# MG-RAST/Shock

Measured on AMD Instinct MI355X. Metric: device-resident index-build GiB/s + Mrecords/s, 10 GiB FASTQ, 1/2/4/8 GPU, higher is better.
Workload: dtype u8; 1 GPU; fastq record index, 10 GiB synthetic node file in HBM (BASELINE configs[1]); records=30969274, bytes=10737418240, tile=16384, parallelism=single slab, exchange=none (one slab: no collective)

## Files before the change

shock_amd/core.py:

```python
from __future__ import annotations

import ctypes
import os
import weakref
from dataclasses import dataclass, field

import numpy as np

from . import _lib as L


@dataclass
class IndexResult:
    count: int
    fmt: str | None
    status: int
    err: bytes | None
    rows: np.ndarray | None = None
    timings: dict = field(default_factory=dict)
    path: int = 0
    reruns: int = 0
    state_out: int = 0
    term_code: int = 0
    flags: int = 0
# ... 157 lines not shown
    def chunkrecord_buffer(self, data: "DeviceBuffer", n: int, rows: "DeviceBuffer", fmt=None,
                           chunk: int = 0) -> IndexResult:
        return self.chunkrecord_device(data.ptr, n, rows.ptr, rows.nbytes // 16, fmt, chunk)

    @staticmethod
    def chunkrecord_capacity(n: int, chunk: int = 0) -> int:
        return n // ((chunk or 1048576) - 32767) + 2

    def column_device(self, d_data: int, n: int, column: int, d_rows: int, row_cap: int) -> IndexResult:
        res = L.Result()
        rc = self._lib.shockidx_column_device(self._h, d_data, n, column, d_rows, row_cap, ctypes.byref(res))
        return _result(res, rc)

    def column_buffer(self, data: "DeviceBuffer", n: int, column: int, rows: "DeviceBuffer") -> IndexResult:
        return self.column_device(data.ptr, n, column, rows.ptr, rows.nbytes // 16)

    def column_fd(self, fd: int, size: int, column: int) -> IndexResult:
        res = L.Result()
        rows_p = ctypes.POINTER(ctypes.c_uint64)()
        rc = self._lib.shockidx_column_fd(self._h, fd, size, column, ctypes.byref(rows_p), ctypes.byref(res))
        rows = _take_rows(rows_p, int(res.count)) if rows_p else None
        return _result(res, rc, rows)

    def column_host(self, data, column: int) -> IndexResult:
        data = bytes(data)
        n = len(data)
        d_in = self.alloc(n + 64)
        d_in.upload(data)
        cap = 1024
        d_rows = self.alloc(16 * cap)
        try:
            r = self.column_buffer(d_in, n, column, d_rows)
            if r.status == L.ESPACE:
                d_rows.free()
                cap = r.count
                d_rows = self.alloc(16 * cap)
                r = self.column_buffer(d_in, n, column, d_rows)
            if r.status == L.OK:
                r.rows = d_rows.rows(r.count) if r.count else np.zeros((0, 2), np.uint64)
            return r
        finally:
            d_in.free()
            d_rows.free()

    def set_dev_cap(self, nbytes: int) -> None:
        rc = self._lib.shockidx_ctx_set_dev_cap(self._h, int(nbytes))
        if rc != 0:
            raise L.ShockIdxError(rc, "shockidx_ctx_set_dev_cap failed")

    def trim(self, keep_bytes: int = 0) -> None:
        rc = self._lib.shockidx_ctx_trim(self._h, int(keep_bytes))
        if rc != L.OK:
            raise L.ShockIdxError(rc, "shockidx_ctx_trim failed")

    def workspace_bytes(self) -> int:
        return int(self._lib.shockidx_ctx_workspace_bytes(self._h))

    def alloc(self, nbytes: int, node: bool = False) -> "DeviceBuffer":
        return DeviceBuffer(self, nbytes, node)

    def sync(self):
        rc = self._lib.shockidx_sync(self._h)
        if rc != L.OK:
            raise L.ShockIdxError(rc, "shockidx_sync failed")

    @property
    def stream(self) -> int:
        return self._lib.shockidx_stream(self._h)

    def subset_index(self, d_ids: int, ids_len: int, d_parent: int, parent_count: int, ilength: int, d_rows: int,
                     rows_cap: int, d_runs: int, runs_cap: int) -> SubsetResult:
        r = L.SubsetResult()
        rc = self._lib.shockidx_subset_index(self._h, d_ids, ids_len, d_parent, parent_count, ilength, d_rows, rows_cap,
                                             d_runs, runs_cap, ctypes.byref(r))
        return _sub_result(r, rc)

    def subset_gather(self, d_data: int, data_len: int, d_runs: int, nruns: int, d_out: int,
                      out_cap: int) -> SubsetResult:
        r = L.SubsetResult()
        rc = self._lib.shockidx_subset_gather(self._h, d_data, data_len, d_runs, nruns, d_out, out_cap,
                                              ctypes.byref(r))
        return _sub_result(r, rc)

    def subset_node(self, d_ids: int, ids_len: int, d_parent: int, parent_count: int, ilength: int, d_rows: int,
                    rows_cap: int, d_runs: int, runs_cap: int, d_data: int, data_len: int, d_out: int,
                    out_cap: int) -> SubsetResult:
        r = L.SubsetResult()
        rc = self._lib.shockidx_subset_node(self._h, d_ids, ids_len, d_parent, parent_count, ilength, d_rows, rows_cap,
                                            d_runs, runs_cap, d_data, data_len, d_out, out_cap, ctypes.byref(r))
        return _sub_result(r, rc)

    def subset_host(self, ids, parent_rows, ilength=None, data=None) -> SubsetResult:
        ids = bytes(ids)
        par = np.ascontiguousarray(parent_rows, dtype=np.uint64).reshape(-1, 2)
        n = par.shape[0]
        il = n if ilength is None else int(ilength)
        d_ids = self.alloc(len(ids) + 64)
        d_ids.upload(ids)
        d_par = self.alloc(16 * n + 64)
        if n:
            d_par.upload(par.tobytes())
        cap = max(1, len(ids) // 2 + 2)
        d_rows = self.alloc(16 * cap)
        d_runs = self.alloc(16 * cap)
        r = self.subset_index(d_ids.ptr, len(ids), d_par.ptr, n, il, d_rows.ptr, cap, d_runs.ptr, cap)
        if r.status in (L.OK, L.EFORMAT):
# ... 338 lines not shown
```

shock_amd/csrc/sidx_build.cpp:

```cpp
#include <errno.h>
#include <hip/hip_runtime.h>
#include <stdio.h>
#include <stdlib.h>
#include <string.h>
#include <sys/mman.h>
#include <unistd.h>

#include <atomic>
#include <mutex>
#include <vector>

#include "../../include/shockidx.h"
#include "sidx_common.hpp"
#include "sidx_subset.hpp"
#include "sidx_launch.hpp"
#include "sidx_host.hpp"

using namespace sidx;

namespace sidx_host {

CopyPool::CopyPool(int n) : nt_(n) {
  for (int i = 0; i < n; ++i) th_.emplace_back([this, i] { run(i); });
}
// ... 167 lines not shown
}

int run_index(shockidx_ctx *c, const uint8_t *d_data, u64 n, int kfmt, u64 *d_rows, u64 row_cap,
              hipStream_t s, DevResult *dr, shockidx_result *res, const SlabGeom *geom, bool general,
              const int *gate) {
  const u64 ntiles = n ? (n + TILE - 1) / TILE : 1;
  if (ntiles >= (1ull << KEY_TILE_BITS)) return set_msg(res, SHOCKIDX_EINVAL, "input too large for one slab");
  if (int rc = ensure_tiles(c, ntiles, res)) return rc;
  const TilePass pass = choose_pass(c, kfmt, n, geom, general);
  if (pass != TP_TWO_PASS) {
    const u64 words = sidx_tile_stage_words(pass, ntiles, c->tiles_grid);
    c->d_tile_stage.node = ws_contig(2);
    if (int rc = c->d_tile_stage.ensure(words, res)) return rc;
    if (int rc = c->d_tile_words.ensure(ntiles * FQ_TILE_WORDS, res)) return rc;
    if (pass == TP_FQ && c->want_spans)
      if (int rc = c->d_fqlines.ensure(ntiles * 3 * (TILE / 64), res)) return rc;
  }
  if (getenv("SHOCKIDX_TIMING") && !c->d_timing) {
    HIPCHK(hipMalloc(&c->d_timing, 9 * 8 * 65536), "hipMalloc(timing)");
  }
  if (c->slots_dirty) {
    HIPCHK(hipMemsetAsync(c->d_small + SMALL_BADKEY, 0xFF, 16, s), "slot reset");
    HIPCHK(hipMemsetAsync(c->d_small + SMALL_COUNTERS, 0, 2 * 4 * NCOUNTERS, s), "slot reset");
    c->slots_dirty = false;
  }
  if (++c->epoch > EPOCH_MASK) {
    HIPCHK(hipMemsetAsync(c->d_status, 0, c->d_status.bytes(), s), "status clear");
    c->epoch = 2;
  }
  c->slots_dirty = true;
  const u32 slot = c->epoch & 1;
  SlabParams p;
  memset(&p, 0, sizeof p);
  p.data = d_data;
  p.n = n;
  p.end = geom ? geom->end : n;
  p.front = geom ? geom->front : 0;
  p.base = geom ? geom->base : 0;
  p.state_in = geom ? geom->state_in : 0;
  p.row_base = geom ? geom->row_base : 0;
  p.summary = geom ? (u64 *)geom->d_summary : nullptr;
  p.row_cap = row_cap;
  p.rows = d_rows;
  auto status_array = [c](StatusArray a) { return c->d_status + (u64)a * c->tiles_cap(); };
  p.status = status_array(SA_STATUS);
  p.pcnt = status_array(SA_PCNT);
  p.ppre = status_array(SA_PPRE);
  for (int i = 0; i < 2; ++i) p.scan_look[i] = status_array((StatusArray)(SA_LOOK0 + i));
  p.tile_agg = status_array(SA_TILE_AGG);
  p.tile_excl = status_array(SA_TILE_EXCL);
  p.pgrid = c->tiles_grid < ntiles ? c->tiles_grid : (u32)ntiles;
  p.fix = general ? nullptr : c->d_fix.get();
  p.fixcap = (u32)c->tiles_cap();
  p.badkey = (u64 *)(c->d_small + SMALL_BADKEY + 8 * slot);
  p.badkey_next = (u64 *)(c->d_small + SMALL_BADKEY + 8 * (slot ^ 1));
  p.detail = c->d_detail;
  p.counters = (u32 *)(c->d_small + SMALL_COUNTERS + 4 * NCOUNTERS * slot);
  p.counters_next = (u32 *)(c->d_small + SMALL_COUNTERS + 4 * NCOUNTERS * (slot ^ 1));
  p.ntiles = (u32)ntiles;
  p.epoch = c->epoch;
  p.seq = geom ? geom->seq : 0;
  p.inject = (c->inject & 4) ? 1u : 0u;
  p.eof = geom ? geom->eof : 1;
  p.file_start = geom ? geom->file_start : 1;
  p.gate = gate;
  p.gate_fmt = kfmt;
  if (const char *dbg = getenv("SHOCKIDX_DEBUG")) p.debug = (u32)atoi(dbg);
  if (getenv("SHOCKIDX_TIMING")) {
    HIPCHK(hipMemsetAsync(c->d_timing, 0, 9 * 8 * 65536, s), "timing clear");
    p.timing = c->d_timing;
  }
  DevResult *d_res = (DevResult *)(c->d_small + SMALL_RESULT);
  const bool tile_pass = pass != TP_TWO_PASS;
  if (tile_pass) {
    p.tile_stage = c->d_tile_stage;
    p.tile_words = c->d_tile_words;
  }
  p.fq_lines = (pass == TP_FQ && c->want_spans) ? c->d_fqlines.get() : nullptr;
  c->last_spans = false;
  std::unique_lock<std::mutex> device_lock(device_mutex(c->device));
  hipEvent_t k0 = tile_pass ? c->ev0 : c->ek0;
  if (!tile_pass) HIPCHK(hipEventRecord(c->ev0, s), "event");
  static const char *const what[] = {"index launch", "tile pass launch", "FASTA tile pass launch",
                                     "line tile pass launch", "SAM tile pass launch"};
  HIPCHK(sidx_launch_tiles(pass, &p, d_res, s, k0, c->ek1), what[pass]);
  if (res) res->path = tile_pass ? 1u : 2u;
  HIPCHK(hipEventRecord(c->ev1, s), "event");
  if (d_rows && verify_rows()) HIPCHK(sidx_launch_verify_rows(d_rows, p.row_base, row_cap, d_res, s), "verify launch");
  HIPCHK(hipMemcpyAsync(c->h_res, d_res, sizeof(DevResult), hipMemcpyDeviceToHost, s), "result copy");
  HIPCHK(hipStreamSynchronize(s), "index sync");
  c->slots_dirty = false;
  if (p.fq_lines) {
    c->last_p = p;
    c->last_spans = true;
  }
  float ms = 0.f;
  (void)hipEventElapsedTime(&ms, c->ev0, c->ev1);
  if (res) res->kernel_ms += ms;
  float kms = 0.f;
  (void)hipEventElapsedTime(&kms, k0, c->ek1);
  if (res) res->index_ms = kms;
  *dr = *c->h_res;
  device_lock.unlock();
  if ((dr->flags & RF_FIXQUEUE) && !general) {
    if (res) res->reruns++;
    return run_index(c, d_data, n, kfmt, d_rows, row_cap, s, dr, res, geom, true, gate);
// ... 262 lines not shown
```

shock_amd/csrc/sidx_capi.cpp:

```cpp
#include <errno.h>
#include <fcntl.h>
#include <hip/hip_runtime.h>
#include <stdio.h>
#include <stdlib.h>
#include <string.h>
#include <unistd.h>

#include <atomic>
#include <random>
#include <string>
#include <thread>

#include <rccl/rccl.h>

#include "../../include/shockidx.h"
#include "sidx_common.hpp"
#include "sidx_subset.hpp"
#include "sidx_launch.hpp"
#include "sidx_slabwalk.hpp"
#include "sidx_host.hpp"

using namespace sidx;
using namespace sidx_host;

// ... 338 lines not shown
}

int shockidx_dev_alloc_node(shockidx_ctx *c, uint64_t bytes, void **d_ptr) {
  if (!c || !d_ptr) return SHOCKIDX_EINVAL;
  if (hipSetDevice(c->device) != hipSuccess) return SHOCKIDX_EHIP;
  return dev_malloc(d_ptr, bytes ? bytes : 16, true) == hipSuccess ? SHOCKIDX_OK : SHOCKIDX_ENOMEM;
}

int shockidx_dev_free(shockidx_ctx *c, void *d_ptr) {
  if (!c) return SHOCKIDX_EINVAL;
  if (hipSetDevice(c->device) != hipSuccess) return SHOCKIDX_EHIP;
  return hipFree(d_ptr) == hipSuccess ? SHOCKIDX_OK : SHOCKIDX_EHIP;
}

int shockidx_memcpy_h2d(shockidx_ctx *c, void *d_dst, const void *src, uint64_t bytes) {
  if (!c) return SHOCKIDX_EINVAL;
  if (hipSetDevice(c->device) != hipSuccess) return SHOCKIDX_EHIP;
  if (hipMemcpyAsync(d_dst, src, bytes, hipMemcpyHostToDevice, c->stream) != hipSuccess) return SHOCKIDX_EHIP;
  return hipStreamSynchronize(c->stream) == hipSuccess ? SHOCKIDX_OK : SHOCKIDX_EHIP;
}

int shockidx_memcpy_d2h(shockidx_ctx *c, void *dst, const void *d_src, uint64_t bytes) {
  if (!c) return SHOCKIDX_EINVAL;
  if (hipSetDevice(c->device) != hipSuccess) return SHOCKIDX_EHIP;
  if (hipMemcpyAsync(dst, d_src, bytes, hipMemcpyDeviceToHost, c->stream) != hipSuccess) return SHOCKIDX_EHIP;
  return hipStreamSynchronize(c->stream) == hipSuccess ? SHOCKIDX_OK : SHOCKIDX_EHIP;
}

int shockidx_memset(shockidx_ctx *c, void *d_dst, int value, uint64_t bytes) {
  if (!c) return SHOCKIDX_EINVAL;
  if (hipSetDevice(c->device) != hipSuccess) return SHOCKIDX_EHIP;
  if (hipMemsetAsync(d_dst, value, bytes, c->stream) != hipSuccess) return SHOCKIDX_EHIP;
  return hipStreamSynchronize(c->stream) == hipSuccess ? SHOCKIDX_OK : SHOCKIDX_EHIP;
}

int shockidx_sync(shockidx_ctx *c) {
  if (!c) return SHOCKIDX_EINVAL;
  if (hipSetDevice(c->device) != hipSuccess) return SHOCKIDX_EHIP;
  return hipDeviceSynchronize() == hipSuccess ? SHOCKIDX_OK : SHOCKIDX_EHIP;
}

void *shockidx_stream(shockidx_ctx *c) { return c ? (void *)c->stream : nullptr; }

int shockidx_debug_timing(shockidx_ctx *c, uint64_t *out, uint32_t nwg) {
  if (!c || !c->d_timing || !out || nwg > 65536) return SHOCKIDX_EINVAL;
  if (hipSetDevice(c->device) != hipSuccess) return SHOCKIDX_EHIP;
  if (hipDeviceSynchronize() != hipSuccess) return SHOCKIDX_EHIP;
  return hipMemcpy(out, c->d_timing, 9 * 8 * (size_t)nwg, hipMemcpyDeviceToHost) == hipSuccess ? SHOCKIDX_OK
                                                                                              : SHOCKIDX_EHIP;
}

int shockidx_debug_tiles_grid(shockidx_ctx *c) { return c ? (int)c->tiles_grid : 0; }

int shockidx_debug_inject(shockidx_ctx *c, uint32_t flags) {
  if (!c) return SHOCKIDX_EINVAL;
  const int old = (int)c->inject;
  c->inject = flags;
  return old;
}

int shockidx_slab_guess(shockidx_ctx *c, const shockidx_slab *sl, int fmt, uint64_t *guess) {
  const Err res;
  if (!c || !sl || !guess) return SHOCKIDX_EINVAL;
  if (sl->is_first) { *guess = 0; return SHOCKIDX_OK; }
  HIPCHK(hipSetDevice(c->device), "hipSetDevice");
  hipStream_t s = c->stream;
  u64 *d_out = (u64 *)(c->d_small + SMALL_DETECT + 32);
  HIPCHK(sidx_launch_slab_guess((const uint8_t *)sl->d_data, sl->n, sl->front, fmt, d_out, s), "guess launch");
  HIPCHK(hipMemcpyAsync(c->h_det + 2, d_out, 8, hipMemcpyDeviceToHost, s), "guess copy");
  HIPCHK(hipStreamSynchronize(s), "guess sync");
  memcpy(guess, c->h_det + 2, 8);
  return SHOCKIDX_OK;
}

int shockidx_slab_index(shockidx_ctx *c, const shockidx_slab *sl, int fmt, uint64_t state_in, void *d_rows,
                        uint64_t row_cap, void *d_summary, shockidx_result *res) {
  shockidx_result tmp;
  if (!res) res = &tmp;
  reset_result(res);
  const bool empty = sl && sl->n == 0 && !sl->is_first;
  if (!c || !sl || !d_summary || (!empty && ((uintptr_t)sl->d_data & 15)) || sl->end < sl->n ||
      (!sl->is_first && sl->n > 0 && sl->front < 16))
    return set_msg(res, SHOCKIDX_EINVAL, "invalid slab");
  if (fmt < SHOCKIDX_FMT_FASTA || fmt > SHOCKIDX_FMT_LINE) return set_msg(res, SHOCKIDX_EINVAL, "invalid format");
  const double t0 = now_ms();
  HIPCHK(hipSetDevice(c->device), "hipSetDevice");
  SlabGeom g;
  g.n = sl->n;
  g.end = empty ? 0 : sl->end;
  g.front = (sl->is_first || empty) ? 0 : sl->front;
  g.base = sl->base;
  g.state_in = state_in;
  g.row_base = sl->is_first ? 0 : 1;
  g.eof = sl->is_last;
  g.file_start = sl->is_first;
  g.d_summary = d_summary;
  g.seq = sl->seq;
  res->format = fmt;
  DevResult dr;
  if (int rc = run_index(c, (const uint8_t *)sl->d_data, sl->n, fmt, (u64 *)d_rows, row_cap, c->stream, &dr, res, &g))
    return rc;
  res->count = dr.count;
  res->state_out = dr.state_out;
  res->term_code = dr.code;
  res->flags = dr.flags;
  res->fixups = dr.fixups;
// ... 95 lines not shown
```

shock_amd/csrc/sidx_common.hpp:

```cpp
#pragma once
#include <stdint.h>

namespace sidx {

typedef unsigned long long u64;
typedef long long i64;
typedef unsigned int u32;

#ifndef SIDX_TILE
#define SIDX_TILE 16384
#endif
#ifndef SIDX_NTHREADS
#define SIDX_NTHREADS (SIDX_TILE / 128)
#endif
constexpr int TILE = SIDX_TILE;
constexpr int NTHREADS = SIDX_NTHREADS;
constexpr int NWAVES = NTHREADS / 64;
constexpr int CHUNK = 16;
constexpr int NCHUNKS = TILE / CHUNK;
constexpr int CPT = NCHUNKS / NTHREADS;
constexpr int REGION = TILE / NTHREADS;
constexpr int MAX_DEFER = 16;
constexpr int FQ_TILE_WORDS = 2 * MAX_DEFER;
#ifndef SIDX_HALO
// ... 17 lines not shown
  ST_FQ_IDMISMATCH = 8,
  ST_FQ_LENMISMATCH = 9,
  ST_FA_INVALID = 10,
  ST_DONTCARE = 11,
  ST_NEEDMORE = 12,
  ST_ABSENT = 13,
  ST_DEFER = 14,
  ST_SLOW = 15,
};

constexpr u64 FLAG_AGG = 1ull << 62;
constexpr u64 FLAG_INC = 2ull << 62;
constexpr int EPOCH_SHIFT = 48;
constexpr u32 EPOCH_MASK = 0x3FFF;
constexpr u64 PAYLOAD_MASK = (1ull << EPOCH_SHIFT) - 1;

constexpr int KEY_TILE_BITS = 24;
constexpr int KEY_REC_SHIFT = 4 + KEY_TILE_BITS;
constexpr u64 KEY_NONE = ~0ull;
constexpr int NCOUNTERS = 8;

enum TilePass : int { TP_TWO_PASS = 0, TP_FQ, TP_FA, TP_LINE, TP_SAM };

struct SlabParams {
  const uint8_t *data;
  u64 n;
  u64 end;
  u64 base;
  u64 state_in;
  u64 row_base;
  u64 row_cap;
  u64 *rows;
  u64 *status;
  u64 *badkey;
  u64 *detail;
  u32 *counters;
  u64 *badkey_next;
  u32 *counters_next;
  u32 ntiles;
  u32 epoch;
  int eof;
  int file_start;
  u64 *timing;
  u64 *summary;
  u64 front;
  u32 debug;
  u64 *pcnt;
  u64 *ppre;
  u64 *scan_look[2];
  u32 pgrid;
  u32 seq;
  u64 *fix;
  u32 fixcap;
  const u64 *tile_excl;
  u64 *tile_agg;
  u32 *tile_stage;
  u32 *tile_words;
  const int *gate;
  int gate_fmt;
  u32 inject;
  uint16_t *fq_lines;
};

struct SlabSummary {
  u64 agg, state_in, key, natural, row_base, err_pos, err_len;
  uint16_t fmt, flags;
  u32 seq;
};
static_assert(sizeof(SlabSummary) == 64, "summary is exchanged as 64 bytes");

struct SlabPlan {
  u64 state_in, first_record, count, err_pos, err_len;
  u32 code;
  int err_rank;
  u32 inconsistent, flags;
};

constexpr u32 RF_CAPACITY = 1;
constexpr u32 RF_INTERNAL = 2;
constexpr u32 RF_HALO = 4;
constexpr u32 RF_FIXQUEUE = 8;
constexpr u32 RF_MISSPEC = 16;

struct ColKey {
  u64 off, lo, len;
};
enum ColCtl : int { COL_BAD = 0, COL_NB, COL_B, COL_CTL_WORDS };

struct DevResult {
  u64 count;
  u64 state_out;
  u64 slab_agg;
  u64 key;
  u64 natural;
  u64 err_pos;
  u64 err_len;
  u32 code;
  u32 flags;
  u32 path;
  u32 fmt;
  u32 fixups;
  u32 fix_tiles;
  u32 detected;
  u32 pad;
};

// ... 2 lines not shown
```

shock_amd/csrc/sidx_host.hpp:

```cpp
#pragma once
#include <hip/hip_runtime.h>
#include <stdint.h>
#include <string.h>

#include <chrono>
#include <condition_variable>
#include <functional>
#include <mutex>
#include <string>
#include <thread>
#include <vector>

#include "../../include/shockidx.h"
#include "sidx_common.hpp"
#include "sidx_devbuf.hpp"

namespace sidx_host {

constexpr size_t STAGE_BYTES = 64ull << 20;
constexpr int NSTAGE = 2;
constexpr size_t SMALL_BADKEY = 0, SMALL_COUNTERS = 64, SMALL_RESULT = 128, SMALL_DETECT = 320, SMALL_CHUNK = 384,
                 SMALL_SLABSUM = 448, SMALL_BYTES = 512;
enum StatusArray : int { SA_STATUS, SA_PCNT, SA_PPRE, SA_LOOK0, SA_LOOK1, SA_TILE_AGG, SA_TILE_EXCL, STATUS_ARRAYS };

inline double now_ms() {
  return std::chrono::duration<double, std::milli>(std::chrono::steady_clock::now().time_since_epoch()).count();
}

class CopyPool {
 public:
  explicit CopyPool(int n);
  ~CopyPool();
  void copy(void *dst, const void *src, size_t n);
  void parallel(size_t n, const std::function<void(size_t, size_t)> &f);

 private:
  void run(int i);
  const int nt_;
  std::vector<std::thread> th_;
  std::mutex m_;
  std::condition_variable cv_, done_;
  const std::function<void(size_t, size_t)> *fn_ = nullptr;
  size_t n_ = 0;
  int pending_ = 0;
  unsigned long long gen_ = 0;
  bool stop_ = false;
};

}

namespace sidx_host {
hipError_t dev_malloc(void **p, size_t bytes, bool node);
const DevAlloc *hip_allocator();
}

struct shockidx_ctx {
  typedef sidx::u64 u64;
  typedef sidx::u32 u32;
  template <class T, size_t PER = 1> using Buf = sidx_host::DevBuf<T, PER>;
  typedef sidx_host::BufClass BufClass;
  int device = 0;
  hipStream_t stream = nullptr;
  hipEvent_t ev0 = nullptr, ev1 = nullptr, ek0 = nullptr, ek1 = nullptr;
  hipEvent_t stage_ev[sidx_host::NSTAGE] = {nullptr, nullptr};
  sidx_host::BufSet bufs{sidx_host::hip_allocator()};
  Buf<uint8_t> d_in{bufs, BufClass::Large, true};
  Buf<u64, 2> d_rows{bufs};
  Buf<u64> d_status{bufs, BufClass::Tile, false, "hipMalloc(status)"};
  Buf<u64> d_detail{bufs, BufClass::Tile, false, "hipMalloc(detail)"};
  Buf<u64> d_fix{bufs, BufClass::Tile, false, "hipMalloc(fix)"};
  u64 tiles_cap() const { return d_fix.cap / 4; }
  uint8_t *d_small = nullptr;
  u32 epoch = 0;
  bool slots_dirty = false;
  int spec_fmt = 0;
  u64 *d_timing = nullptr;
  u32 tiles_grid = 0;
  uint8_t *h_stage[sidx_host::NSTAGE] = {nullptr, nullptr};
  sidx::DevResult *h_res = nullptr;
  sidx_host::CopyPool *pool = nullptr;
  Buf<uint8_t> d_sub{bufs};
  int *h_det = nullptr;
  u64 ws_cap = 0;
  u64 dev_cap = 0;
  Buf<u32> d_tile_stage{bufs};
  Buf<u32> d_tile_words{bufs};
  Buf<uint8_t> d_cra{bufs};
  Buf<uint8_t> d_crb{bufs};
  Buf<uint8_t> d_slot[2] = {Buf<uint8_t>{bufs, BufClass::Large, true, "hipMalloc(slab slot)"},
                            Buf<uint8_t>{bufs, BufClass::Large, true, "hipMalloc(slab slot)"}};
  u32 cr_grid = 0;
  Buf<uint8_t> d_cola{bufs};
  Buf<uint8_t> d_colb{bufs};
  Buf<uint8_t> d_plan{bufs};
  Buf<uint8_t> d_sec{bufs};
  hipStream_t s_copy = nullptr;
  uint8_t *h_rows[2] = {nullptr, nullptr};
  bool want_spans = false;
  Buf<uint16_t> d_fqlines{bufs};
  sidx::SlabParams last_p;
  bool last_spans = false;
  u32 inject = 0;
};

namespace sidx_host {

int set_hip(Err r, hipError_t e, const char *what);
template <class R> void reset_result(R *r) {
  if (r) memset(r, 0, sizeof *r);
}
const char *status_message(uint32_t code);

#define HIPCHK(expr, what)                      \
  do {                                          \
    hipError_t _e = (expr);                     \
    if (_e != hipSuccess) return sidx_host::set_hip(res, _e, what); \
  } while (0)

template <class Read>
int fasta_error_text(Err res, uint64_t err_len, Read read_piece) {
  static const char pre[] = "Invalid fasta entry: ";
  char text[sizeof pre - 1 + 50];
  const uint64_t show = err_len < 50 ? err_len : 50;
  memcpy(text, pre, sizeof pre - 1);
  if (show)
    if (int rc = read_piece(text + sizeof pre - 1, show)) return rc;
  return set_msg(res, SHOCKIDX_EFORMAT, text, sizeof pre - 1 + show);
}

struct Carver {
// ... 95 lines not shown
```

shock_amd/csrc/sidx_kernels.hip:

```cpp
#include <hip/hip_runtime.h>
#include <hip/hip_ext.h>
#include <atomic>

#include "sidx_common.hpp"
#include "sidx_device.hpp"
#include "sidx_launch.hpp"
#include "sidx_stage.hpp"

namespace sidx {

constexpr u64 INF = ~0ull;

#ifndef SIDX_DIAG
#define SIDX_DIAG 0
#endif
__device__ __forceinline__ u32 dbg(const SlabParams &p) { return SIDX_DIAG ? p.debug : 0u; }
__device__ __forceinline__ u64 *tmg(const SlabParams &p) { return SIDX_DIAG ? p.timing : nullptr; }

__device__ __forceinline__ u32 fr_to_st(u32 r) { return r == FR_DEFER ? ST_DEFER : ST_NEEDMORE; }

template <class A>
__device__ u32 fastq_record(A &a, u64 s, u64 &len) {
  u64 e0, e1, e2, e3;
  u32 r;
  if (s >= a.end) return a.eof ? ST_END : ST_NEEDMORE;
  r = a.find(C_NL, s, INF, e0);
  if (r >= FR_DEFER) return fr_to_st(r);
  if (r == FR_NONE) return ST_FQ_TRUNC;
  if (e0 == s) {
    if ((s >= 4 || a.front >= 4) && a.byte(s - 1) == '\n' && a.byte(s - 2) == '\n' &&
        a.byte(s - 3) == '\n' && a.byte(s - 4) == '\n')
      return ST_DONTCARE;
    u64 y, z;
    r = a.find(C_NOTNL, s, INF, y);
    if (r >= FR_DEFER) return fr_to_st(r);
    if (r == FR_NONE) return ST_END;
    r = a.find(C_NL, y, INF, z);
    if (r >= FR_DEFER) return fr_to_st(r);
    return r == FR_FOUND ? ST_FQ_EMPTYLINES : ST_FQ_TRUNC;
  }
  if (a.byte(s) != '@') return ST_FQ_NOAT;
  if (e0 - s == 1) return ST_FQ_NOID;
  r = a.find(C_NL, e0 + 1, INF, e1);
  if (r >= FR_DEFER) return fr_to_st(r);
  if (r == FR_NONE) return ST_FQ_TRUNC;
  if (e1 == e0 + 1) return ST_FQ_EMPTYSEQ;
  r = a.find(C_NL, e1 + 1, INF, e2);
  if (r >= FR_DEFER) return fr_to_st(r);
  if (r == FR_NONE) return ST_FQ_TRUNC;
  if (a.byte(e1 + 1) != '+') return ST_FQ_NOPLUS;
  u64 plo, phi;
  trim_space(a, e1 + 1, e2 + 1, plo, phi);
  if (phi - plo > 1) {
    u64 ilo, ihi;
    trim_space(a, s + 1, e0 + 1, ilo, ihi);
    if (ihi - ilo != phi - plo - 1) return ST_FQ_IDMISMATCH;
// ... 693 lines not shown
__device__ __forceinline__ u32 lds_diff4(const uint8_t *raw, u32 a, u32 b, u32 n) {
  const u32 *w = reinterpret_cast<const u32 *>(raw);
  const u32 wa = __builtin_amdgcn_alignbyte(w[(a >> 2) + 1], w[a >> 2], a & 3);
  const u32 wb = __builtin_amdgcn_alignbyte(w[(b >> 2) + 1], w[b >> 2], b & 3);
  const u32 m = n >= 4 ? ~0u : ((1u << (8 * n)) - 1u);
  return (wa ^ wb) & m;
}


#pragma clang diagnostic ignored "-Wbitwise-instead-of-logical"
__device__ __forceinline__ bool fq_ok(const uint8_t *r, u32 s, u32 e0, u32 e1, u32 e2, u32 e3, u32 &cn, u32 &cb,
                                      u32 &crs, bool &idclean) {
  const u32 cs = r[s], ci1 = r[s + 1], cs1 = r[e0 + 1], cp = r[e1 + 1], cq1 = r[e2 + 1];
  const u32 a0 = r[e0 - 1], a1 = r[e1 - 1], a2 = r[e2 - 1], a3 = r[e3 - 1];
  const u32 b0 = r[e0 - 2], b1 = r[e1 - 2], b2 = r[e2 - 2], b3 = r[e3 - 2];
  const u32 c0 = a0 == '\r', c1 = a1 == '\r', c2 = a2 == '\r', c3 = a3 == '\r';
  const u32 z0 = e0 - c0, z1 = e1 - c1, z2 = e2 - c2, z3 = e3 - c3;
  const u32 l0 = c0 ? b0 : a0, l1 = c1 ? b1 : a1, l2 = c2 ? b2 : a2, l3 = c3 ? b3 : a3;
  const bool pluslong = z2 > e1 + 2;
  const bool ok = (e0 > s + 1) & (cs == '@') & (cp == '+') &
                  (z1 > e0 + 1) & ascii_nonspace(cs1) & ascii_nonspace(l1) &
                  (z3 > e2 + 1) & ascii_nonspace(cq1) & ascii_nonspace(l3) &
                  (z1 - e0 == z3 - e2) &
                  ascii_nonspace(l2) &
                  (!pluslong | (ascii_nonspace(ci1) & ascii_nonspace(l0) & (z0 - s == z2 - e1 - 1)));
  cn = (ok && pluslong) ? z0 - s - 1 : 0u;
  cb = e1 + 2;
  crs = c0 | (c1 << 1) | (c3 << 2);
  idclean = ascii_nonspace(ci1) & ascii_nonspace(l0) & (z0 > s + 1);
  return ok;
}

__device__ __forceinline__ u32 fq_guess_at(const uint8_t *raw, const uint16_t *nlpos, u32 TT, int lane) {
  const u32 c = (u32)lane & 15u;
  const u32 a = nlpos[c], b1 = nlpos[c + 1], b2 = nlpos[c + 2], b3 = nlpos[c + 3], b4 = nlpos[c + 4];
  const u32 x = raw[FRONT + a + 1], y = raw[FRONT + b2 + 1];
  const bool ok = ((u32)lane < 16) & (c + 4 < TT) & (x == '@') & (y == '+') & (b2 - b1 > 1) & ((b2 - b1) == (b4 - b3));
  const u64 m = __ballot(ok);
  return m ? (ctz64(m) & 3u) : GUESS_NONE;
}

typedef __attribute__((address_space(1))) u32 gu32;
__device__ __forceinline__ u32 g_add(u32 *p, u32 v) {
  return __hip_atomic_fetch_add((gu32 *)p, v, __ATOMIC_RELAXED, __HIP_MEMORY_SCOPE_AGENT);
}
__device__ __forceinline__ void g_or(u32 *p, u32 v) {
  (void)__hip_atomic_fetch_or((gu32 *)p, v, __ATOMIC_RELAXED, __HIP_MEMORY_SCOPE_AGENT);
}
__device__ __forceinline__ void g_min64(u64 *p, u64 v) {
  (void)__hip_atomic_fetch_min((__attribute__((address_space(1))) u64 *)p, v, __ATOMIC_RELAXED,
                               __HIP_MEMORY_SCOPE_AGENT);
}

__device__ __forceinline__ void push_fix(const SlabParams &p, u64 start, u64 g, u32 tile) {
  const u32 i = g_add(&p.counters[2], 1u);
  if (i < p.fixcap) {
    gu64 *f = (gu64 *)(p.fix + (sizeof(FixRec) / sizeof(u64)) * (u64)i);
    f[0] = start; f[1] = g; f[2] = tile;
  } else {
    g_or(&p.counters[3], 1u);
  }
  if (start == ~0ull) (void)g_add(&p.counters[3], 2u);
}


constexpr u32 FQ_LINE_E = 64;
constexpr u32 FQ_OVF = ((RCAP + 1 - FQ_LINE_E) + 7u) & ~7u;
__device__ __forceinline__ u64 fq_ovf(const SlabParams &p, u64 t) { return (u64)p.ntiles * FQ_LINE_E + t * FQ_OVF; }
__device__ __forceinline__ u32 fq_start(const SlabParams &p, u64 t, u32 L) {
  const uint16_t *s = reinterpret_cast<const uint16_t *>(p.tile_stage);
  return L < FQ_LINE_E ? s[t * FQ_LINE_E + L] : s[fq_ovf(p, t) + (L - FQ_LINE_E)];
}
constexpr u32 FQ_UNCERT = 0x8000;
__device__ __forceinline__ u32 *fq_defer(const SlabParams &p, u64 t) { return p.tile_words + t * (2 * MAX_DEFER); }

constexpr u32 FQ_BLK = 16;
constexpr u64 FQ_RR = 32;
static_assert(FQ_RR % FQ_BLK == 0, "a batch holds whole bursts");
struct __align__(16) TilesSmem {
  uint16_t nlpos[SNLCAP + 8];
  uint16_t line[FQ_BLK][FQ_LINE_E];
  u64 words[FQ_BLK];
  u32 wtot[SNW];
  u32 nh, ndefer, slow, pad;
};

__device__ __forceinline__ void fq_put(const SlabParams &p, TilesSmem &S, u64 t, u32 j, u32 L, uint16_t v) {
  if (L < FQ_LINE_E) S.line[j][L] = v;
  else __builtin_nontemporal_store(v, reinterpret_cast<uint16_t *>(p.tile_stage) + fq_ovf(p, t) + (L - FQ_LINE_E));
}

template <bool kSpans>
__device__ __forceinline__ void tiles_iter(const SlabParams &p, TilesSmem &S, uint8_t *raw, u64 t, int tid, int lane,
                                           int wid, u64 *tacc, u32 j, bool flush) {
  u64 tprev = tacc ? stamp() : 0;
#define TILES_STAMP(i)              \
  if (tacc) {                       \
    const u64 tn_ = stamp();        \
    tacc[i] += tn_ - tprev;         \
    tprev = tn_;                    \
  }
  __builtin_amdgcn_s_setprio(3);
  stage_tile<true>(p, t, (u32)(size_t)(lds_u8 *)raw, wid, lane);
  __builtin_amdgcn_s_setprio(0);
  asm volatile("s_waitcnt vmcnt(0)" ::: "memory");
  TILES_STAMP(0);
  if (wid == SNW - 1) __builtin_amdgcn_s_setprio(1);
  const u64 tlo = t * TILE;
  const u64 thi = (tlo + TILE < p.n) ? tlo + TILE : p.n;
  const u32 tlen = (u32)(thi - tlo);
  const u32 llen = (u32)(((tlo + TILE + SHALO < p.end) ? tlo + TILE + SHALO : p.end) - tlo);
  if (llen < (u32)(TILE + SHALO) || (t == 0 && p.front < FRONT)) {
    lds_barrier();
    for (u32 c = (u32)tid; c < (u32)((TILE + SHALO) / 16); c += SNT) {
      const u32 o = c * 16;
      if (o + 16 <= llen) continue;
      uint4 v = make_uint4(0, 0, 0, 0);
      if (o < llen) {
        v = keep_bytes(*reinterpret_cast<const uint4 *>(raw + FRONT + o), llen - o);
        if (llen & 3u) {
          u32 ll;
          const auto rs = tile_rsrc(p, t, ll);
          patch_tail(v, o, llen, tail_dword(rs, llen));
        }
      }
      *reinterpret_cast<uint4 *>(raw + FRONT + o) = v;
    }
    if (t == 0 && p.front < FRONT && tid == 0) *reinterpret_cast<uint4 *>(raw) = make_uint4(0, 0, 0, 0);
    lds_barrier();
  }
  u64 m = 0;
// ... 148 lines not shown
        uint16_t *ln = p.fq_lines + t * (3 * RCAP) + 3 * L;
        ln[0] = (uint16_t)(idclean ? (e0 | ((crs & 1u) << 15)) : 0xFFFFu);
        ln[1] = (uint16_t)(e1 | ((crs & 2u) << 14));
        ln[2] = (uint16_t)(e2 | ((crs & 4u) << 13));
      }
      if (L + 1 == nrec && known) fq_put(p, S, t, j, nrec, (uint16_t)(e3 + 1));
      if (!good && !dontcare) {
        const u32 slot = atomicAdd(&S.ndefer, 1u);
        if (slot < (u32)MAX_DEFER) { tdef[slot] = L; tdef[MAX_DEFER + slot] = s0; }
        else S.slow = 1;
      }
    }
  }
  __builtin_amdgcn_s_setprio(0);
  TILES_STAMP(3);
  lds_barrier();
  TILES_STAMP(4);
  const u64 word = fq_word(T, gi0, nrec, slow || S.slow, S.ndefer < (u32)MAX_DEFER ? S.ndefer : (u32)MAX_DEFER);
  typedef unsigned v4u __attribute__((ext_vector_type(4)));
  {
    if (tid == 0) S.words[j] = word;
    if (flush && wid == 0) {
      asm volatile("s_waitcnt lgkmcnt(0)" ::: "memory");
      const u64 t0 = t - j;
      for (u32 c = (u32)lane; c < (j + 1) * (FQ_LINE_E / 8); c += 64) {
        const v4u v = *reinterpret_cast<const v4u *>(&S.line[0][0] + 8 * c);
        __builtin_nontemporal_store(v, (__attribute__((address_space(1))) v4u *)(reinterpret_cast<uint16_t *>(p.tile_stage) +
                                                                                 t0 * FQ_LINE_E + 8 * c));
      }
      if ((u32)lane * 2 < j + 1) {
        if ((u32)lane * 2 + 1 < j + 1) {
          const v4u v = *reinterpret_cast<const v4u *>(&S.words[2 * lane]);
          *(__attribute__((address_space(1))) v4u *)(p.tile_agg + t0 + 2 * lane) = v;
        } else {
          p.tile_agg[t0 + 2 * lane] = S.words[2 * lane];
        }
      }
    }
  }
  TILES_STAMP(5);
#undef TILES_STAMP
}

#ifndef SIDX_TILES_WGS
#define SIDX_TILES_WGS 7
#endif
template <bool kSpans>
__global__ __launch_bounds__(SNT, SIDX_TILES_WGS) void k_fq_tiles(const SlabParams p) {
  __shared__ __attribute__((aligned(16))) uint8_t raw[SSLOT];
  __shared__ TilesSmem S;
  if (gated_off(p)) return;
  const int tid = threadIdx.x, lane = tid & 63;
  const int wid = __builtin_amdgcn_readfirstlane(tid >> 6);
  const u64 G = p.pgrid;
  u64 tacc_[8] = {0, 0, 0, 0, 0, 0, 0, 0};
  u64 *tacc = (tmg(p) && (tid == 0 || tid == 64)) ? tacc_ : nullptr;
  u64 ntl = 0;
  const u64 nbat = (p.ntiles + FQ_RR - 1) / FQ_RR;
  for (u64 c = blockIdx.x; c < nbat; c += G) {
    const u64 tb = c * FQ_RR, te = tb + FQ_RR < p.ntiles ? tb + FQ_RR : p.ntiles;
    for (u64 t = tb; t < te; ++t) {
      const u32 j = (u32)(t - tb) & (FQ_BLK - 1);
      tiles_iter<kSpans>(p, S, raw, t, tid, lane, wid, tacc, j, j == FQ_BLK - 1 || t + 1 == te);
      ++ntl;
    }
  }
  if (tacc) {
    u64 *o = tmg(p) + ((u64)blockIdx.x * 2 + (tid ? 1 : 0)) * 9;
    for (int i = 0; i < 8; ++i) o[i] = tacc[i];
    o[8] = ntl;
  }
}

constexpr u32 LCAP = TILE / 16;
constexpr u64 LOFF_SHIFT = 32, LCOUNT = (1ull << LOFF_SHIFT) - 1;
#ifndef SIDX_LINE_WGS
#define SIDX_LINE_WGS 7
#endif
__global__ __launch_bounds__(SNT, SIDX_LINE_WGS) void k_line_tiles(const SlabParams p) {
  __shared__ __attribute__((aligned(16))) uint8_t raw[FRONT + TILE];
  __shared__ __attribute__((aligned(16))) uint16_t sp[LCAP];
  __shared__ u32 wtot[SNW], wlast[SNW];
  const int tid = threadIdx.x, lane = tid & 63;
  const int wid = __builtin_amdgcn_readfirstlane(tid >> 6);
  const u64 G = p.pgrid;
  u64 t = first_tile(blockIdx.x, G);
  uint4 *stage16 = reinterpret_cast<uint4 *>(p.tile_stage);
  u64 wofs = (t * (p.ntiles / G) + (t < p.ntiles % G ? t : p.ntiles % G)) * (LCAP / 8);
  u64 pt = ~0ull, pword = 0, ppcnt = 0, pwofs = 0;
  u32 pT = 0;
  auto flush_pending = [&]() -> u32 {
    if (pt == ~0ull) return 0u;
    u32 n = 0;
    if (wid == 0) {
      if (tid == 0) {
        p.tile_agg[pt] = pword;
        p.pcnt[pt] = ppcnt;
      }
      n = 2;
    }
    if (pT <= LCAP && (u32)wid * 512u < pT) {
      if ((u32)tid * 8 < pT) {
        typedef unsigned v4u_t __attribute__((ext_vector_type(4)));
        const uint4 x = *reinterpret_cast<const uint4 *>(&sp[8 * tid]);
        *reinterpret_cast<v4u_t *>(stage16 + pwofs + (u64)tid) = (v4u_t){x.x, x.y, x.z, x.w};
      }
      ++n;
    }
    pt = ~0ull;
    return n;
  };
  for (; t < p.ntiles; t += G) {
    __builtin_amdgcn_s_setprio(3);
    stage_tile<false>(p, t, (u32)(size_t)(lds_u8 *)raw, wid, lane);
    __builtin_amdgcn_s_setprio(0);
    {
      const u32 nst = flush_pending();
      if (nst == 0) asm volatile("s_waitcnt vmcnt(0)" ::: "memory");
      else if (nst == 1) asm volatile("s_waitcnt vmcnt(1)" ::: "memory");
// ... 696 lines not shown
  lds_barrier();
  __builtin_amdgcn_s_setprio(2);
  const bool slow = ncand > (u32)RCAP;
  uint16_t *stage = reinterpret_cast<uint16_t *>(p.tile_stage + t * RCAP);
  const bool own0 = p.file_start || t != 0;
  const u32 skip0 = own0 ? ~0u : ((delta && !(p.state_in & 1)) ? 1u : 0u);
  if (!slow) {
    for (u32 i = (u32)tid; i < ncand; i += SNT) {
      const u32 c = S.cand[i];
      const u32 g = c & 0x3FFFu, lo = c >> 14;
      u32 st;
      if (i == skip0) st = FA_SKIP;
      else if (i == 0 && delta) st = FA_DEFER;
      else st = fa_check(r, S.mnl, lo, g, lo == 0 && (t != 0 || !p.file_start));
      stage[i] = (uint16_t)(g | (st << 14));
      if (st == FA_INV) atomicMin(&S.finv, i);
    }
  }
  u32 *tw = p.tile_words + t * FAW;
  if (tid == SNT - 1) {
    const u32 wi = alast >> 6;
    const u64 w0 = wi < (u32)(TILE / 64) ? S.mnl[wi] & (~0ull << (alast & 63)) : 0ull;
    const u64 w1 = wi + 1 < (u32)(TILE / 64) ? S.mnl[wi + 1] : 0ull;
    u32 q = w0 ? (wi << 6) + ctz64(w0) : (w1 ? ((wi + 1) << 6) + ctz64(w1) : fa_find_nl(S.mnl, alast, tlen));
    if (q > tlen) q = tlen;
    S.tcert = (q > alast && q + 1 < tlen && ascii_nonspace(r[q - 1]) && ascii_nonspace(r[q + 1])) ? 1u : 0u;
  }
  if (t == p.ntiles - 1 && tid == SNT - 1) {
    u32 est = FA_OK;
    const u32 lo = alast;
    if (p.end > p.n || !p.eof) {
    } else if (lo != 0 || (t == 0 && p.file_start)) {
      if (tlen > lo + 1 && fa_find_nl(S.mnl, lo, tlen) < tlen) est = fa_check(r, S.mnl, lo, tlen, false);
    } else {
      est = fa_check(r, S.mnl, 0, tlen, true);
    }
    tw[6] = est;
    tw[7] = lo;
  }
  __builtin_amdgcn_s_setprio(0);
  lds_barrier();
  {
    const u32 finv = S.finv;
    const u64 word = fa_word(A, ncand, slow, delta, delta ? (S.cand[0] & 0x3FFFu) : FA_NONE,
                             (A >> 3) ? (S.cand[delta] & 0x3FFFu) : FA_NONE, finv != FA_NONE, S.tcert != 0);
    if (tid == 0) p.tile_agg[t] = word;
    if (tid == 0 && finv != FA_NONE) {
      tw[4] = finv;
      tw[5] = S.cand[finv] >> 14;
    }
  }
}

constexpr u64 FA_RR = 32;
#ifndef SIDX_FA_WGS
#define SIDX_FA_WGS 7
#endif
__global__ __launch_bounds__(SNT, SIDX_FA_WGS) void k_fa_tiles(const SlabParams p) {
  __shared__ __attribute__((aligned(16))) uint8_t raw[FRONT + TILE];
  __shared__ FaSmem S;
  if (gated_off(p)) return;
  const int tid = threadIdx.x, lane = tid & 63;
  const int wid = __builtin_amdgcn_readfirstlane(tid >> 6);
  const u64 G = p.pgrid;
  const u64 nbat = (p.ntiles + FA_RR - 1) / FA_RR;
  for (u64 c = blockIdx.x; c < nbat; c += G) {
    const u64 tb = c * FA_RR, te = tb + FA_RR < p.ntiles ? tb + FA_RR : p.ntiles;
    for (u64 t = tb; t < te; ++t) fa_iter(p, S, raw, t, tid, lane, wid);
  }
}

__device__ __forceinline__ u32 fa_first(u32 flags, u32 fc, u32 fd, u64 st) {
  return ((flags & 2) && (st & 1)) ? fc : fd;
}
__device__ u64 fa_next_global(const SlabParams &p, u64 u, int lane) {
  for (; u < p.ntiles; u += 64) {
    const u64 v = u + (u64)lane;
    u32 f = FA_NONE;
    if (v < p.ntiles) {
      const u64 w = p.tile_agg[v];
      f = fa_first(fa_w_flags(w), fa_w_fc(w), fa_w_fd(w), FastaMonoid::apply(p.state_in, p.tile_excl[v]));
    }
    const u64 bal = __ballot(f != FA_NONE);
    if (bal) {
      const int L = (int)ctz64(bal);
      return (u + (u64)L) * TILE + (u32)__shfl((int)f, L, 64);
    }
  }
  return p.n;
}

__global__ __launch_bounds__(256) void k_fa_place(const SlabParams p) {
  __shared__ uint4 sw[PLACE_TILES + 1][2];
  __shared__ u64 sS[PLACE_TILES + 1];
  __shared__ u32 sC[PLACE_TILES];
  if (gated_off(p)) return;
  const int tid = threadIdx.x, lane = tid & 63, wid = tid >> 6;
  for (u64 t0 = (u64)blockIdx.x * PLACE_TILES; t0 < p.ntiles; t0 += (u64)gridDim.x * PLACE_TILES) {
    if (tid >= 128 && tid < 128 + PLACE_TILES) {
      const u64 u = t0 + (u64)(tid - 128);
      sC[tid - 128] = (u >= 1 && u - 1 < p.ntiles) ? (u32)fa_w_tcert(p.tile_agg[u - 1]) : 0u;
    }
    if (tid <= PLACE_TILES && t0 + tid < p.ntiles) {
      const u64 w = p.tile_agg[t0 + tid];
      const u32 *tw = p.tile_words + (t0 + tid) * FAW;
      const bool last = t0 + tid == p.ntiles - 1;
      sw[tid][0] = make_uint4((u32)(w >> 18) & 0xFFFu, fa_w_flags(w), fa_w_fc(w), fa_w_fd(w));
      sw[tid][1] = make_uint4((w >> 63) ? tw[4] : FA_NONE, (w >> 63) ? tw[5] : 0u, last ? tw[6] : FA_OK,
                              last ? tw[7] : 0u);
      sS[tid] = FastaMonoid::apply(p.state_in, p.tile_excl[t0 + tid]);
    }
    __syncthreads();
    const int sub = lane >> 4, sl = lane & 15;
    for (int kb = wid * 4; kb < PLACE_TILES; kb += 16) {
      const int k = kb + sub;
      const u64 t = t0 + k;
      const bool live = t < p.ntiles;
      if (!__ballot(live)) break;
      const uint4 w0 = sw[k][0], w1 = sw[k][1];
      const u32 ncand = w0.x, flags = w0.y, finv = w1.x, invlo = w1.y, est = w1.z, elo = w1.w;
      const u64 st = sS[k];
      const u64 cnt = st >> 1;
// ... 458 lines not shown
  if (e != hipSuccess) return e;
  if (ek1) (void)hipEventRecord(ek1, s);
  return finalize(p, F, d_res, s);
}

constexpr u32 FIX_GRID = 64;
hipError_t launch_fq(const SlabParams &p, DevResult *d_res, hipStream_t s, hipEvent_t ek0, hipEvent_t ek1) {
  if (p.fq_lines) hipExtLaunchKernelGGL(k_fq_tiles<true>, dim3(p.pgrid), dim3(SNT), 0, s, ek0, ek1, 0, p);
  else hipExtLaunchKernelGGL(k_fq_tiles<false>, dim3(p.pgrid), dim3(SNT), 0, s, ek0, ek1, 0, p);
  hipError_t e = scan_excl<CountMonoid>(p, p.tile_agg, (u64 *)p.tile_excl, 0, true, s, FQW_TMASK);
  if (e != hipSuccess) return e;
  if (p.debug & 4096u) return hipErrorLaunchFailure;
  hipLaunchKernelGGL(k_fq_place, dim3(place_grid(p.ntiles, PLACE_TILES)), dim3(256), 0, s, p);
  hipLaunchKernelGGL(k_fixup, dim3(FIX_GRID), dim3(256), 0, s, p, d_res);
  return hipGetLastError();
}

hipError_t launch_fa(const SlabParams &p, DevResult *d_res, hipStream_t s, hipEvent_t ek0, hipEvent_t ek1) {
  hipExtLaunchKernelGGL(k_fa_tiles, dim3(p.pgrid), dim3(SNT), 0, s, ek0, ek1, 0, p);
  hipError_t e = scan_excl<FastaMonoid>(p, p.tile_agg, (u64 *)p.tile_excl, 0, true, s, FAW_AMASK);
  if (e != hipSuccess) return e;
  hipLaunchKernelGGL(k_fa_place, dim3(place_grid(p.ntiles, PLACE_TILES)), dim3(256), 0, s, p);
  hipLaunchKernelGGL(k_fa_fixup, dim3(FIX_GRID), dim3(256), 0, s, p, d_res);
  return hipGetLastError();
}

hipError_t launch_line(const SlabParams &p, DevResult *d_res, hipStream_t s, hipEvent_t ek0, hipEvent_t ek1) {
  hipExtLaunchKernelGGL(k_line_tiles, dim3(p.pgrid), dim3(SNT), 0, s, ek0, ek1, 0, p);
  hipError_t e = scan_excl<CountMonoid>(p, p.tile_agg, (u64 *)p.tile_excl, 0, true, s, LCOUNT);
  if (e == hipSuccess) e = scan_excl<MaxMonoid>(p, p.pcnt, p.ppre, 1, false, s);
  if (e != hipSuccess) return e;
  hipLaunchKernelGGL(k_line_place<F_LINE>, dim3(place_grid(p.ntiles, LPLACE_TILES)), dim3(256), 0, s, p);
  hipLaunchKernelGGL(k_line_final, dim3(1), dim3(64), 0, s, p);
  return finalize(p, F_LINE, d_res, s);
}

hipError_t launch_sam(const SlabParams &p, DevResult *d_res, hipStream_t s, hipEvent_t ek0, hipEvent_t ek1) {
  hipExtLaunchKernelGGL(k_sam_tiles, dim3(p.pgrid), dim3(SNT), 0, s, ek0, ek1, 0, p);
  hipError_t e = scan_excl<SamMonoid>(p, p.tile_agg, (u64 *)p.tile_excl, 0, true, s);
  if (e != hipSuccess) return e;
  hipLaunchKernelGGL(k_sam_resolve, dim3((p.ntiles + 255) / 256), dim3(256), 0, s, p);
  e = scan_excl<MaxMonoid>(p, p.pcnt, p.ppre, 1, false, s);
  if (e != hipSuccess) return e;
  hipLaunchKernelGGL(k_line_place<F_SAM>, dim3(place_grid(p.ntiles, LPLACE_TILES)), dim3(256), 0, s, p);
  hipLaunchKernelGGL(k_sam_final, dim3(1), dim3(64), 0, s, p);
  return finalize(p, F_SAM, d_res, s);
}
}

extern "C" hipError_t sidx_launch_tiles(TilePass pass, const SlabParams *pp, DevResult *d_res, hipStream_t s,
                                        hipEvent_t ek0, hipEvent_t ek1) {
  SlabParams p = *pp;
  if (pass == TP_FA || pass == TP_LINE || pass == TP_SAM) p.pgrid = tile_grid(p, pass);
  switch (pass) {
    case TP_FQ: return launch_fq(p, d_res, s, ek0, ek1);
    case TP_FA: return launch_fa(p, d_res, s, ek0, ek1);
    case TP_LINE: return launch_line(p, d_res, s, ek0, ek1);
    case TP_SAM: return launch_sam(p, d_res, s, ek0, ek1);
    case TP_TWO_PASS:
      switch (p.gate_fmt) {
        case F_FASTQ: return launch_two_pass<F_FASTQ>(p, d_res, s, ek0, ek1);
        case F_FASTA: return launch_two_pass<F_FASTA>(p, d_res, s, ek0, ek1);
        case F_SAM: return launch_two_pass<F_SAM>(p, d_res, s, ek0, ek1);
        case F_LINE: return launch_two_pass<F_LINE>(p, d_res, s, ek0, ek1);
      }
  }
  return hipErrorInvalidValue;
}

static_assert(FQ_LINE_E + FQ_OVF <= 2 * RCAP, "a FASTQ tile's starts fit its slot");
extern "C" u64 sidx_tile_stage_words(TilePass pass, u64 ntiles, u32 grid) {
  return (pass == TP_LINE || pass == TP_SAM) ? ntiles * (LCAP / 2) : (ntiles + grid + 16) * (u64)RCAP;
}

extern "C" hipError_t sidx_launch_fq_spans_place(const SlabParams *pp, u32 *spans, u64 *outlen, u64 K, int kind,
                                                hipStream_t s) {
  const SlabParams &p = *pp;
  if (!p.fq_lines || !p.ntiles) return hipSuccess;
  hipLaunchKernelGGL(k_fq_spans_place, dim3(place_grid(p.ntiles, 4)), dim3(256), 0, s, p, spans, outlen, K, kind);
  return hipGetLastError();
}

extern "C" int sidx_tiles_blocks_per_cu() {
  int n = 0;
  return hipOccupancyMaxActiveBlocksPerMultiprocessor(&n, k_fq_tiles<false>, SNT, 0) == hipSuccess ? n : 0;
}
```

Baseline: 4588 GiB/s.

## Replace static round-robin tile batches with dynamic atomic claims and finer tail

The FASTQ and FASTA tile kernels stop striding over fixed 32-tile batches by block index and instead claim batches dynamically through an atomic counter. The counter is fetched a few tiles before the current claim ends so its latency is hidden. A claim plan shrinks the batch size when there are few tiles per block and splits the final batches into smaller ones to even out the tail. A debug hook to cap the grid is also added. The aim is to cut load imbalance at the end of the kernel, at the cost of one atomic per claim and a dependence on the counter being reset between launches.

```diff
diff --git a/shock_amd/core.py b/shock_amd/core.py
--- a/shock_amd/core.py
+++ b/shock_amd/core.py
@@ -233,6 +233,13 @@
         rc = self._lib.shockidx_ctx_trim(self._h, int(keep_bytes))
         if rc != L.OK:
             raise L.ShockIdxError(rc, "shockidx_ctx_trim failed")
+
+    def debug_set_tiles_grid(self, g: int) -> None:
+        fn = self._lib.shockidx_debug_set_tiles_grid
+        fn.argtypes, fn.restype = [ctypes.c_void_p, ctypes.c_int], ctypes.c_int
+        rc = fn(self._h, int(g))
+        if rc != L.OK:
+            raise L.ShockIdxError(rc, "shockidx_debug_set_tiles_grid failed (after the first build, or g out of range)")
 
     def workspace_bytes(self) -> int:
         return int(self._lib.shockidx_ctx_workspace_bytes(self._h))
diff --git a/shock_amd/csrc/sidx_build.cpp b/shock_amd/csrc/sidx_build.cpp
--- a/shock_amd/csrc/sidx_build.cpp
+++ b/shock_amd/csrc/sidx_build.cpp
@@ -243,6 +243,7 @@
   p.pgrid = c->tiles_grid < ntiles ? c->tiles_grid : (u32)ntiles;
   p.fix = general ? nullptr : c->d_fix.get();
   p.fixcap = (u32)c->tiles_cap();
+  p.grid_cap = c->grid_cap;
   p.badkey = (u64 *)(c->d_small + SMALL_BADKEY + 8 * slot);
   p.badkey_next = (u64 *)(c->d_small + SMALL_BADKEY + 8 * (slot ^ 1));
   p.detail = c->d_detail;
diff --git a/shock_amd/csrc/sidx_capi.cpp b/shock_amd/csrc/sidx_capi.cpp
--- a/shock_amd/csrc/sidx_capi.cpp
+++ b/shock_amd/csrc/sidx_capi.cpp
@@ -414,6 +414,12 @@
 
 int shockidx_debug_tiles_grid(shockidx_ctx *c) { return c ? (int)c->tiles_grid : 0; }
 
+int shockidx_debug_set_tiles_grid(shockidx_ctx *c, int g) {
+  if (!c || c->epoch != 0 || g < 1 || (u32)g > c->tiles_grid) return SHOCKIDX_EINVAL;
+  c->tiles_grid = c->grid_cap = (u32)g;
+  return SHOCKIDX_OK;
+}
+
 int shockidx_debug_inject(shockidx_ctx *c, uint32_t flags) {
   if (!c) return SHOCKIDX_EINVAL;
   const int old = (int)c->inject;
diff --git a/shock_amd/csrc/sidx_claim.hpp b/shock_amd/csrc/sidx_claim.hpp
--- /dev/null
+++ b/shock_amd/csrc/sidx_claim.hpp
@@ -0,0 +1,59 @@
+#pragma once
+#include <stdint.h>
+
+#if defined(__HIPCC__)
+#define SIDX_CLAIM_HD __host__ __device__ inline
+#else
+#define SIDX_CLAIM_HD inline
+#endif
+
+namespace sidx {
+
+#ifndef CLAIM_TAIL_DIV
+#define CLAIM_TAIL_DIV 2
+#endif
+static_assert(CLAIM_TAIL_DIV == 1 || CLAIM_TAIL_DIV == 2 || CLAIM_TAIL_DIV == 4, "the tail's claims: B, B/2 or B/4 tiles");
+constexpr uint32_t CLAIM_BMAX = 32;
+constexpr uint32_t CLAIM_BMIN = 2;
+
+struct ClaimPlan {
+  uint32_t B;
+  uint32_t nmain;
+  uint32_t tail_b;
+  uint32_t tail_t0;
+  uint32_t nclaims;
+  uint32_t ntiles;
+};
+struct ClaimRange {
+  uint32_t tb, te;
+};
+
+SIDX_CLAIM_HD ClaimPlan claim_plan(uint32_t ntiles, uint32_t G) {
+  uint32_t B = CLAIM_BMAX;
+  while (B > CLAIM_BMIN && (uint64_t)((ntiles + B - 1) / B) < 4ull * G) B >>= 1;
+  const uint32_t nb = (ntiles + B - 1) / B;
+  ClaimPlan pl;
+  pl.B = B;
+  pl.nmain = nb > G ? nb - G : 0u;
+  pl.tail_b = B / CLAIM_TAIL_DIV > CLAIM_BMIN ? B / CLAIM_TAIL_DIV : CLAIM_BMIN;
+  pl.tail_t0 = pl.nmain * B;
+  pl.nclaims = pl.nmain + (ntiles - pl.tail_t0 + pl.tail_b - 1) / pl.tail_b;
+  pl.ntiles = ntiles;
+  return pl;
+}
+
+SIDX_CLAIM_HD ClaimRange claim_range(const ClaimPlan &pl, uint32_t c) {
+  ClaimRange r;
+  if (c < pl.nmain) {
+    r.tb = c * pl.B;
+    r.te = r.tb + pl.B;
+  } else if (c < pl.nclaims) {
+    r.tb = pl.tail_t0 + (c - pl.nmain) * pl.tail_b;
+    r.te = pl.ntiles - r.tb > pl.tail_b ? r.tb + pl.tail_b : pl.ntiles;
+  } else {
+    r.tb = r.te = pl.ntiles;
+  }
+  return r;
+}
+
+}
diff --git a/shock_amd/csrc/sidx_common.hpp b/shock_amd/csrc/sidx_common.hpp
--- a/shock_amd/csrc/sidx_common.hpp
+++ b/shock_amd/csrc/sidx_common.hpp
@@ -93,6 +93,7 @@
   u32 seq;
   u64 *fix;
   u32 fixcap;
+  u32 grid_cap;
   const u64 *tile_excl;
   u64 *tile_agg;
   u32 *tile_stage;
diff --git a/shock_amd/csrc/sidx_host.hpp b/shock_amd/csrc/sidx_host.hpp
--- a/shock_amd/csrc/sidx_host.hpp
+++ b/shock_amd/csrc/sidx_host.hpp
@@ -76,6 +76,7 @@
   int spec_fmt = 0;
   u64 *d_timing = nullptr;
   u32 tiles_grid = 0;
+  u32 grid_cap = 0;
   uint8_t *h_stage[sidx_host::NSTAGE] = {nullptr, nullptr};
   sidx::DevResult *h_res = nullptr;
   sidx_host::CopyPool *pool = nullptr;
diff --git a/shock_amd/csrc/sidx_kernels.hip b/shock_amd/csrc/sidx_kernels.hip
--- a/shock_amd/csrc/sidx_kernels.hip
+++ b/shock_amd/csrc/sidx_kernels.hip
@@ -2,6 +2,7 @@
 #include <hip/hip_ext.h>
 #include <atomic>
 
+#include "sidx_claim.hpp"
 #include "sidx_common.hpp"
 #include "sidx_device.hpp"
 #include "sidx_launch.hpp"
@@ -801,6 +802,31 @@
                                __HIP_MEMORY_SCOPE_AGENT);
 }
 
+constexpr u32 CLAIM_AHEAD = 8;
+template <class Body>
+__device__ __forceinline__ void claim_loop(const SlabParams &p, u32 &word, int tid, Body &&body) {
+  const ClaimPlan cp = claim_plan(p.ntiles, p.pgrid);
+  u32 nx = 0;
+  for (u32 c = blockIdx.x; c < cp.nclaims;) {
+    const ClaimRange r = claim_range(cp, c);
+    const bool more = c + 1 < cp.nclaims;
+    const u32 ta = r.te - r.tb > CLAIM_AHEAD ? r.te - CLAIM_AHEAD : r.tb;
+    for (u32 t = r.tb; t < r.te; ++t) {
+      if (more && tid == 0) {
+        if (t == ta) {
+          u32 z = 0;
+          asm("" : "+v"(z));
+          nx = g_add(&p.counters[6] + z, 1u);
+        }
+        if (t == ta + 1) word = nx;
+      }
+      body(t, r);
+    }
+    if (!more) break;
+    c = p.pgrid + (u32)__builtin_amdgcn_readfirstlane((int)word);
+  }
+}
+
 __device__ __forceinline__ void push_fix(const SlabParams &p, u64 start, u64 g, u32 tile) {
   const u32 i = g_add(&p.counters[2], 1u);
   if (i < p.fixcap) {
@@ -824,8 +850,9 @@
 __device__ __forceinline__ u32 *fq_defer(const SlabParams &p, u64 t) { return p.tile_words + t * (2 * MAX_DEFER); }
 
 constexpr u32 FQ_BLK = 16;
-constexpr u64 FQ_RR = 32;
-static_assert(FQ_RR % FQ_BLK == 0, "a batch holds whole bursts");
+static_assert(CLAIM_BMIN % 2 == 0 && FQ_BLK % 2 == 0,
+              "claims, and so bursts, start at even tiles: the tile words leave 16 bytes per lane");
+static_assert(CLAIM_BMAX <= 32, "a claim holds at most 32 tiles (the batch size measured best)");
 struct __align__(16) TilesSmem {
   uint16_t nlpos[SNLCAP + 8];
   uint16_t line[FQ_BLK][FQ_LINE_E];
@@ -1080,19 +1107,14 @@
   if (gated_off(p)) return;
   const int tid = threadIdx.x, lane = tid & 63;
   const int wid = __builtin_amdgcn_readfirstlane(tid >> 6);
-  const u64 G = p.pgrid;
   u64 tacc_[8] = {0, 0, 0, 0, 0, 0, 0, 0};
   u64 *tacc = (tmg(p) && (tid == 0 || tid == 64)) ? tacc_ : nullptr;
   u64 ntl = 0;
-  const u64 nbat = (p.ntiles + FQ_RR - 1) / FQ_RR;
-  for (u64 c = blockIdx.x; c < nbat; c += G) {
-    const u64 tb = c * FQ_RR, te = tb + FQ_RR < p.ntiles ? tb + FQ_RR : p.ntiles;
-    for (u64 t = tb; t < te; ++t) {
-      const u32 j = (u32)(t - tb) & (FQ_BLK - 1);
-      tiles_iter<kSpans>(p, S, raw, t, tid, lane, wid, tacc, j, j == FQ_BLK - 1 || t + 1 == te);
-      ++ntl;
-    }
-  }
+  claim_loop(p, S.pad, tid, [&](u32 t, const ClaimRange &r) {
+    const u32 j = (t - r.tb) & (FQ_BLK - 1);
+    tiles_iter<kSpans>(p, S, raw, t, tid, lane, wid, tacc, j, j == FQ_BLK - 1 || t + 1 == r.te);
+    ++ntl;
+  });
   if (tacc) {
     u64 *o = tmg(p) + ((u64)blockIdx.x * 2 + (tid ? 1 : 0)) * 9;
     for (int i = 0; i < 8; ++i) o[i] = tacc[i];
@@ -1895,7 +1917,6 @@
   }
 }
 
-constexpr u64 FA_RR = 32;
 #ifndef SIDX_FA_WGS
 #define SIDX_FA_WGS 7
 #endif
@@ -1905,12 +1926,7 @@
   if (gated_off(p)) return;
   const int tid = threadIdx.x, lane = tid & 63;
   const int wid = __builtin_amdgcn_readfirstlane(tid >> 6);
-  const u64 G = p.pgrid;
-  const u64 nbat = (p.ntiles + FA_RR - 1) / FA_RR;
-  for (u64 c = blockIdx.x; c < nbat; c += G) {
-    const u64 tb = c * FA_RR, te = tb + FA_RR < p.ntiles ? tb + FA_RR : p.ntiles;
-    for (u64 t = tb; t < te; ++t) fa_iter(p, S, raw, t, tid, lane, wid);
-  }
+  claim_loop(p, S.pad[0], tid, [&](u32 t, const ClaimRange &) { fa_iter(p, S, raw, t, tid, lane, wid); });
 }
 
 __device__ __forceinline__ u32 fa_first(u32 flags, u32 fc, u32 fd, u64 st) {
@@ -2475,6 +2491,7 @@
                                         hipEvent_t ek0, hipEvent_t ek1) {
   SlabParams p = *pp;
   if (pass == TP_FA || pass == TP_LINE || pass == TP_SAM) p.pgrid = tile_grid(p, pass);
+  if (p.grid_cap && p.pgrid > p.grid_cap) p.pgrid = p.grid_cap;
   switch (pass) {
     case TP_FQ: return launch_fq(p, d_res, s, ek0, ek1);
     case TP_FA: return launch_fa(p, d_res, s, ek0, ek1);
```

New measurement: 4687 GiB/s (median of 6 runs). 2.2% higher.
